# rsjahnige/CRYSTALS-Kyber

Hardware: AMD Instinct MI355X
Metric: ML-KEM-768 encaps+decaps/sec at batch 2^20; achieved HBM GB/s vs peak (higher is better)
Workload: dtype u32+f32 (64-bit Keccak lanes as 2 x u32; mod-3329 arithmetic exact on integers < 2^24 in the fp32 pipe; u8/u16 I/O)

## Files before the change

### crystals-kyber_amd/__init__.py

```python
import ctypes as C
import os

HERE = os.path.dirname(os.path.abspath(__file__))
LIB_PATH = os.environ.get("MLKEM_LIB_PATH") or os.path.join(HERE, "libmlkem_amd.so")
SHIM_PATH = os.path.join(HERE, "libml_kem.so")

SIZES = {512: (800, 1632, 768), 768: (1184, 2400, 1088), 1024: (1568, 3168, 1568)}
ERR_RNG = -2
ERR_MODULUS = -4
ERR_HASH = -5
ERR_KEY = -6
ERR_ARG = -101
KEYCHECK_EK_MODULUS = 1
KEYCHECK_DK_MODULUS = 2
KEYCHECK_DK_HASH = 4
KEYCHECK_EK_MISMATCH = 8
KEYCHECK_SEED = 16
KEYCHECK_PCT = 32

ABI_SYMBOLS = (
    "mlkem_sizes", "mlkem_params", "mlkem_device_count", "mlkem_strerror", "mlkem_last_hip_error",
    "mlkem_ctx_create", "mlkem_ctx_destroy", "mlkem_ctx_scratch_bytes", "mlkem_timing_begin", "mlkem_timing_end",
    "mlkem_keygen_dev", "mlkem_encaps_dev", "mlkem_decaps_dev", "mlkem_encaps_status_dev", "mlkem_ctx_set_conformance", "mlkem_ctx_debug_stages",
    "mlkem_encaps_shared_dev", "mlkem_decaps_shared_dev",
    "mlkem_pke_keygen_dev", "mlkem_pke_encrypt_dev", "mlkem_pke_decrypt_dev",
    "mlkem_ntt_dev", "mlkem_intt_dev", "mlkem_multiply_ntts_dev", "mlkem_sample_ntt_dev", "mlkem_sample_cbd_dev",
    "mlkem_compress_encode_dev", "mlkem_decode_decompress_dev",
    "mlkem_prf_dev", "mlkem_hash_dev", "mlkem_keccak_sponge_dev", "mlkem_sha3_pad_bits",
    "mlkem_keygen", "mlkem_encaps", "mlkem_decaps", "mlkem_ntt", "mlkem_intt", "mlkem_keccak_sponge",
    "mlkem_sample_ntt", "mlkem_sample_ntt_retries", "mlkem_sample_ntt_retries_dev", "mlkem_sample_cbd",
    "mlkem_keygen_random", "mlkem_encaps_random",
    "mlkem_cells_to_bytes_dev", "mlkem_bytes_to_cells_dev", "mlkem_keygen_stream", "mlkem_encaps_stream", "mlkem_decaps_stream", "mlkem_stream_release",
    "mlkem_compress_dev", "mlkem_decompress_dev", "mlkem_compress", "mlkem_decompress", "mlkem_sha3_pad_suffix",
    "mlkem_selftest_count", "mlkem_selftest", "mlkem_host_release", "mlkem_host_register", "mlkem_host_unregister",
    "mlkem_multi_create", "mlkem_multi_destroy", "mlkem_multi_members", "mlkem_multi_device", "mlkem_shard_range",
    "mlkem_keygen_multi", "mlkem_encaps_multi", "mlkem_decaps_multi",
    "mlkem_keygen_multi_dev", "mlkem_encaps_multi_dev", "mlkem_decaps_multi_dev", "mlkem_multi_sync", "mlkem_multi_stream", "mlkem_stream_last_staged",
    "mlkem_vector_multiply_dev", "mlkem_poly_add_dev", "mlkem_poly_sub_dev",
# ... 41 lines not shown
    L.mlkem_check_keys_dev.argtypes = [vp, i32, sz, vp, vp, vp, vp, vp, vp]
    L.mlkem_check_keys.argtypes = [i32, sz, vp, vp, vp, vp, vp]
    L.mlkem_keyset_create.argtypes = [vp, i32, sz, vp, vp, vp, vp, C.POINTER(vp), vp]
    L.mlkem_keyset_destroy.argtypes = [vp]
    L.mlkem_keyset_destroy.restype = None
    L.mlkem_keyset_info.argtypes = [vp, C.POINTER(i32), C.POINTER(sz), C.POINTER(i32), C.POINTER(sz)]
    L.mlkem_encaps_keyset_dev.argtypes = [vp, vp, sz, vp, vp, vp, vp, vp, vp]
    L.mlkem_decaps_keyset_dev.argtypes = [vp, vp, sz, vp, vp, vp, vp, vp]
    L.mlkem_ctx_rng_seed.argtypes = [vp, vp]
    L.mlkem_keygen_random_dev.argtypes = [vp, i32, sz, vp, vp, vp, vp]
    L.mlkem_encaps_random_dev.argtypes = [vp, i32, sz, vp, vp, vp, vp, vp]
    L.mlkem_encaps_keyset_random_dev.argtypes = [vp, vp, sz, vp, vp, vp, vp, vp]
    L.mlkem_encaps_status_dev.argtypes = [vp, i32, sz, vp, vp, vp, vp, vp, vp]
    L.mlkem_ctx_set_conformance.argtypes = [vp, i32]
    L.mlkem_ctx_debug_stages.argtypes = [vp, C.c_uint]
    L.mlkem_encaps_shared_dev.argtypes = [vp, i32, sz, vp, vp, vp, vp, vp]
    L.mlkem_decaps_shared_dev.argtypes = [vp, i32, sz, vp, vp, vp, vp, vp]
    L.mlkem_pke_keygen_dev.argtypes = [vp, i32, sz, vp, vp, vp, vp]
    L.mlkem_pke_encrypt_dev.argtypes = [vp, i32, sz, vp, vp, vp, vp, vp]
    L.mlkem_pke_decrypt_dev.argtypes = [vp, i32, sz, vp, vp, vp, vp]
    L.mlkem_ntt_dev.argtypes = [vp, sz, vp, vp, vp]
    L.mlkem_intt_dev.argtypes = [vp, sz, vp, vp, vp]
    L.mlkem_multiply_ntts_dev.argtypes = [vp, sz, vp, vp, vp, vp]
    L.mlkem_sample_ntt_dev.argtypes = [vp, sz, vp, vp, vp]
    L.mlkem_sample_cbd_dev.argtypes = [vp, i32, sz, vp, vp, vp]
    L.mlkem_prf_dev.argtypes = [vp, i32, sz, vp, vp, vp]
    L.mlkem_compress_encode_dev.argtypes = [vp, i32, sz, vp, vp, vp]
    L.mlkem_decode_decompress_dev.argtypes = [vp, i32, sz, vp, vp, vp]
    L.mlkem_hash_dev.argtypes = [vp, i32, sz, vp, C.c_uint, sz, vp, vp]
    L.mlkem_keygen.argtypes = [i32, sz, vp, vp, vp, vp]
# ... 125 lines not shown
        shape = (n,) if last is None else (n, last)
        if given is None:
            return torch.empty(shape, dtype=dtype, device=self.device)
        if not isinstance(given, torch.Tensor):
            raise MLKEMError(-101, "output must be a torch tensor")
        if given.device != self.device or given.dtype != dtype or tuple(given.shape) != shape or not given.is_contiguous():
            raise MLKEMError(-101, f"output tensor must be contiguous {dtype} {shape} on {self.device}, got "
                                   f"{given.dtype} {tuple(given.shape)} on {given.device}"
                                   f"{'' if given.is_contiguous() else ' (non-contiguous)'}")
        return given

    @property
    def scratch_bytes(self):
        return self.lib.mlkem_ctx_scratch_bytes(self._ctx)

    def keygen(self, d, z, ek=None, dk=None):
        u8 = self.torch.uint8
        d, z = self._dev(d, u8, 32), self._dev(z, u8, 32)
        n = d.shape[0]
        if z.shape[0] != n:
            raise MLKEMError(-101, "d and z batch sizes differ")
        ek = self._out(n, self.ek_len, given=ek)
        dk = self._out(n, self.dk_len, given=dk)
        self._check(self.lib.mlkem_keygen_dev(self._ctx, self.param_set, n, d.data_ptr(), z.data_ptr(), ek.data_ptr(),
                                              dk.data_ptr(), self._stream()))
        return ek, dk

    def encaps(self, ek, m, c=None, K=None, return_status=False):
        u8 = self.torch.uint8
        ek, m = self._dev(ek, u8, self.ek_len), self._dev(m, u8, 32)
# ... 577 lines not shown
```

### crystals-kyber_amd/csrc/mlkem_capi.hip

```cpp
#include "mlkem_pipeline.hpp"
#include "mlkem_keyset.hpp"
#include "mlkem_rng.hpp"
#include "mlkem_selftest.hpp"

#include "../../include/mlkem_batch.h"

#include <sys/random.h>

#include <cstdio>
#include <cstdlib>
#include <cstring>
#include <string.h>
#include <algorithm>
#include <condition_variable>
#include <functional>
#include <map>
#include <memory>
#include <mutex>
#include <new>
#include <string>
#include <thread>
#include <vector>

using namespace mlkem;
// ... 348 lines not shown
    return MLKEM_OK;
}
int mlkem_encaps_dev(mlkem_ctx* ctx, int set, size_t n, const uint8_t* ek, const uint8_t* m, uint8_t* c, uint8_t* K, void* stream) {
    return mlkem_encaps_status_dev(ctx, set, n, ek, m, c, K, nullptr, stream);
}

int mlkem_ctx_set_conformance(mlkem_ctx* ctx, int mode) {
    if (!ctx_ok(ctx) || (mode != MLKEM_CONFORMANCE_REFERENCE && mode != MLKEM_CONFORMANCE_FIPS203)) return MLKEM_ERR_ARG;
    ctx->ws.fips = mode == MLKEM_CONFORMANCE_FIPS203;
    return MLKEM_OK;
}

int mlkem_ctx_debug_stages(mlkem_ctx* ctx, unsigned mask) {
    if (!ctx_ok(ctx) || mask > 15u) return MLKEM_ERR_ARG;
    ctx->ws.stages = mask;
    return MLKEM_OK;
}

int mlkem_decaps_dev(mlkem_ctx* ctx, int set, size_t n, const uint8_t* dk, const uint8_t* c, uint8_t* K, int32_t* status, void* stream) {
    ParamSet p;
    if (!param_set(set, p)) return MLKEM_ERR_PARAM_SET;
    if (!ctx_ok(ctx) || (n && (!dk || !c || !K))) return MLKEM_ERR_ARG;
    if (!aligned16(dk) || !aligned16(c) || !aligned16(K) || (reinterpret_cast<uintptr_t>(status) & 3u)) return MLKEM_ERR_ARG;
    hipStream_t st = static_cast<hipStream_t>(stream);
    ctx_arm_side(ctx, n);
    decaps_dispatch(st, set, n, dk, c, K, status, status != nullptr, ctx->ws);
    HIP_TRY(hipGetLastError());
    return MLKEM_OK;
}

// ... 1421 lines not shown
```

### crystals-kyber_amd/csrc/mlkem_device.hpp

```cpp
#pragma once
#ifndef MLKEM_EMU
#include <hip/hip_runtime.h>
#endif
#include <stdint.h>

namespace mlkem {

constexpr int KQ = 3329;
constexpr int INV128 = 3303;

constexpr int cx_bitrev7(int r) {
    int o = 0;
    for (int i = 0; i < 7; i++) o |= ((r >> i) & 1) << (6 - i);
    return o;
}
constexpr int cx_pow17(int e) {
    int r = 1;
    for (int i = 0; i < e; i++) r = (r * 17) % KQ;
    return r;
}
constexpr int cx_centered(int x) { return x > KQ / 2 ? x - KQ : x; }
__device__ __forceinline__ unsigned div_q(unsigned num) {
    return (unsigned)(((uint64_t)num * 10321340ull) >> 35);
}
// ... 26 lines not shown
template <int N>
__device__ __forceinline__ void rotl64(uint32_t lo, uint32_t hi, uint32_t& olo, uint32_t& ohi) {
    if constexpr (N == 0) {
        olo = lo; ohi = hi;
    } else if constexpr (N < 32) {
        olo = __builtin_amdgcn_alignbit(lo, hi, 32 - N);
        ohi = __builtin_amdgcn_alignbit(hi, lo, 32 - N);
    } else if constexpr (N == 32) {
        olo = hi; ohi = lo;
    } else {
        olo = __builtin_amdgcn_alignbit(hi, lo, 64 - N);
        ohi = __builtin_amdgcn_alignbit(lo, hi, 64 - N);
    }
}

#define MLKEM_RHOPI(dst, src, rot, dx)                                                       \
    {                                                                                        \
        uint32_t tl = MLKEM_XOR3(s.lo[src], cl[(dx + 4) % 5], rl[(dx + 1) % 5]);             \
        uint32_t th = MLKEM_XOR3(s.hi[src], ch[(dx + 4) % 5], rh[(dx + 1) % 5]);             \
        rotl64<rot>(tl, th, bl[dst], bh[dst]);                                               \
    }

__device__ __forceinline__ void keccak_f1600(KeccakState& s) {
#pragma unroll 1
    for (int round = 0; round < 24; round++) {
        uint32_t cl[5], ch[5], rl[5], rh[5], bl[25], bh[25];
#pragma unroll
        for (int x = 0; x < 5; x++) {
            cl[x] = MLKEM_XOR3(MLKEM_XOR3(s.lo[x], s.lo[x + 5], s.lo[x + 10]), s.lo[x + 15], s.lo[x + 20]);
            ch[x] = MLKEM_XOR3(MLKEM_XOR3(s.hi[x], s.hi[x + 5], s.hi[x + 10]), s.hi[x + 15], s.hi[x + 20]);
        }
#pragma unroll
        for (int x = 0; x < 5; x++) rotl64<1>(cl[x], ch[x], rl[x], rh[x]);
        MLKEM_RHOPI(0, 0, 0, 0)   MLKEM_RHOPI(10, 1, 1, 1)  MLKEM_RHOPI(20, 2, 62, 2) MLKEM_RHOPI(5, 3, 28, 3)  MLKEM_RHOPI(15, 4, 27, 4)
        MLKEM_RHOPI(16, 5, 36, 0) MLKEM_RHOPI(1, 6, 44, 1)  MLKEM_RHOPI(11, 7, 6, 2)  MLKEM_RHOPI(21, 8, 55, 3) MLKEM_RHOPI(6, 9, 20, 4)
        MLKEM_RHOPI(7, 10, 3, 0)  MLKEM_RHOPI(17, 11, 10, 1) MLKEM_RHOPI(2, 12, 43, 2) MLKEM_RHOPI(12, 13, 25, 3) MLKEM_RHOPI(22, 14, 39, 4)
        MLKEM_RHOPI(23, 15, 41, 0) MLKEM_RHOPI(8, 16, 45, 1) MLKEM_RHOPI(18, 17, 15, 2) MLKEM_RHOPI(3, 18, 21, 3) MLKEM_RHOPI(13, 19, 8, 4)
        MLKEM_RHOPI(14, 20, 18, 0) MLKEM_RHOPI(24, 21, 2, 1) MLKEM_RHOPI(9, 22, 61, 2) MLKEM_RHOPI(19, 23, 56, 3) MLKEM_RHOPI(4, 24, 14, 4)
#pragma unroll
        for (int y = 0; y < 25; y += 5) {
#pragma unroll
            for (int x = 0; x < 5; x++) {
                s.lo[y + x] = MLKEM_CHI(bl[y + x], bl[y + (x + 1) % 5], bl[y + (x + 2) % 5]);
                s.hi[y + x] = MLKEM_CHI(bh[y + x], bh[y + (x + 1) % 5], bh[y + (x + 2) % 5]);
            }
        }
        s.lo[0] ^= KECCAK_RC[2 * round];
        s.hi[0] ^= KECCAK_RC[2 * round + 1];
    }
}

__device__ __forceinline__ void keccak_zero(KeccakState& s) {
#pragma unroll
    for (int i = 0; i < 25; i++) { s.lo[i] = 0; s.hi[i] = 0; }
}

template <int POS>
__device__ __forceinline__ void keccak_xor_byte(KeccakState& s, uint32_t byte) {
    constexpr int w = POS / 4, sh = 8 * (POS % 4);
    if constexpr (w % 2 == 0) s.lo[w / 2] ^= byte << sh;
    else s.hi[w / 2] ^= byte << sh;
}
template <int W>
// ... 178 lines not shown
```

### crystals-kyber_amd/csrc/mlkem_kernels.hpp

```cpp
#pragma once
#include "mlkem_device.hpp"

namespace mlkem {

constexpr int WAVE = 64;

#ifndef MLKEM_KECCAK_MINWAVES
#define MLKEM_KECCAK_MINWAVES 6
#endif

struct MsgView {
    const uint8_t* p0; size_t stride0; unsigned len0;
    const uint8_t* p1; size_t stride1; unsigned len1;
};

__device__ __forceinline__ uint2 load_qword_tail(const uint8_t* p, unsigned avail) {
    if (avail >= 8) return *reinterpret_cast<const uint2*>(p);
    uint2 v;
    v.x = 0; v.y = 0;
    for (unsigned i = 0; i < avail; i++) {
        const uint32_t b = p[i];
        if (i < 4) v.x |= b << (8 * i);
        else v.y |= b << (8 * (i - 4));
    }
// ... 143 lines not shown
}

__device__ __forceinline__ void keccak_xor_byte_rt(KeccakState& s, unsigned pos, uint32_t byte) {
    const unsigned w = pos >> 2;
    const uint32_t v = byte << (8 * (pos & 3));
#define MLKEM_XB(W) keccak_word<W>(s) ^= (w == W) ? v : 0u;
    MLKEM_XB(0) MLKEM_XB(1) MLKEM_XB(2) MLKEM_XB(3) MLKEM_XB(4) MLKEM_XB(5) MLKEM_XB(6) MLKEM_XB(7)
    MLKEM_XB(8) MLKEM_XB(9) MLKEM_XB(10) MLKEM_XB(11) MLKEM_XB(12) MLKEM_XB(13) MLKEM_XB(14) MLKEM_XB(15)
    MLKEM_XB(16) MLKEM_XB(17) MLKEM_XB(18) MLKEM_XB(19) MLKEM_XB(20) MLKEM_XB(21) MLKEM_XB(22) MLKEM_XB(23)
    MLKEM_XB(24) MLKEM_XB(25) MLKEM_XB(26) MLKEM_XB(27) MLKEM_XB(28) MLKEM_XB(29) MLKEM_XB(30) MLKEM_XB(31)
    MLKEM_XB(32) MLKEM_XB(33) MLKEM_XB(34) MLKEM_XB(35) MLKEM_XB(36) MLKEM_XB(37) MLKEM_XB(38) MLKEM_XB(39)
    MLKEM_XB(40) MLKEM_XB(41)
#undef MLKEM_XB
}

template <int RATE, int SUFFIX>
__device__ __forceinline__ void wave_sponge_absorb(KeccakState& s, uint2* stage, const MsgView& mv, size_t item0,
                                                   size_t n_items) {
    const unsigned total = mv.len0 + mv.len1;
    keccak_zero(s);
#if MLKEM_STAGE_DMA
    if (item0 + WAVE <= n_items && total != 0 && total % 4 == 0 && (mv.len1 == 0 || mv.len0 % 16 == 0) &&
        mv.stride0 < (1u << 27) && mv.stride1 < (1u << 27)) {
        uint32_t* st32 = reinterpret_cast<uint32_t*>(stage);
        const unsigned nfull = total / (unsigned)RATE, rem = total - nfull * (unsigned)RATE;
        wave_dma_half<RATE>(st32, mv, item0, 0, nfull ? (unsigned)RATE : rem, 0);
#pragma unroll 1
        for (unsigned b = 0; b < nfull; b++) {
            wave_absorb_dma<RATE, true>(s, st32, mv, item0, b * RATE, RATE);
            if (b + 1 < nfull) wave_dma_half<RATE>(st32, mv, item0, (b + 1) * RATE, RATE, 0);
            else if (rem) wave_dma_half<RATE>(st32, mv, item0, nfull * RATE, rem, 0);
            keccak_f1600(s);
        }
        if (rem) wave_absorb_dma<RATE, false>(s, st32, mv, item0, nfull * RATE, rem);
        keccak_xor_byte_rt(s, rem, SUFFIX);
        keccak_xor_byte<RATE - 1>(s, 0x80);
        keccak_f1600(s);
        return;
    }
#endif
    unsigned voff = 0;
    while (total - voff >= (unsigned)RATE) {
        wave_absorb_block<RATE>(s, stage, mv, item0, n_items, voff);
        keccak_f1600(s);
        voff += RATE;
    }
    const unsigned rem = total - voff;
    if (rem) wave_absorb_block<RATE>(s, stage, mv, item0, n_items, voff);
    keccak_xor_byte_rt(s, rem, SUFFIX);
    keccak_xor_byte<RATE - 1>(s, 0x80);
    keccak_f1600(s);
}

constexpr int stage_qwords(int max_rate) {
    const int sync_q = STAGE_ROWS * (max_rate / 8);
    const int dma_q = MLKEM_STAGE_DMA ? 2 * ((max_rate / 4 + 3) / 4) * WAVE / 2 : 0;
    return sync_q > dma_q ? sync_q : dma_q;
}
constexpr int STAGE_QWORDS = stage_qwords(168);

__device__ __forceinline__ void store32(uint8_t* base, size_t stride, size_t item, const uint32_t (&w)[8]) {
    uint32_t* p = reinterpret_cast<uint32_t*>(base + item * stride);
#pragma unroll
    for (int i = 0; i < 8; i++) p[i] = w[i];
}
__device__ __forceinline__ void load32(const uint8_t* base, size_t stride, size_t item, uint32_t (&w)[8]) {
// ... 2 lines not shown
    for (int i = 0; i < 8; i++) w[i] = p[i];
}
#define MLKEM_STATE_WORDS8(s, FIRST, w)                                                             \
    {                                                                                               \
        w[0] = keccak_word<FIRST + 0>(s); w[1] = keccak_word<FIRST + 1>(s); w[2] = keccak_word<FIRST + 2>(s); \
        w[3] = keccak_word<FIRST + 3>(s); w[4] = keccak_word<FIRST + 4>(s); w[5] = keccak_word<FIRST + 5>(s); \
        w[6] = keccak_word<FIRST + 6>(s); w[7] = keccak_word<FIRST + 7>(s);                         \
    }
#define MLKEM_SET_WORDS8(s, FIRST, w)                                                               \
    {                                                                                               \
        keccak_word<FIRST + 0>(s) = w[0]; keccak_word<FIRST + 1>(s) = w[1]; keccak_word<FIRST + 2>(s) = w[2]; \
        keccak_word<FIRST + 3>(s) = w[3]; keccak_word<FIRST + 4>(s) = w[4]; keccak_word<FIRST + 5>(s) = w[5]; \
        keccak_word<FIRST + 6>(s) = w[6]; keccak_word<FIRST + 7>(s) = w[7];                         \
    }

__device__ __forceinline__ void lane_G64(KeccakState& s, const uint32_t (&x)[8], const uint32_t (&y)[8]) {
    keccak_zero(s);
    MLKEM_SET_WORDS8(s, 0, x)
    MLKEM_SET_WORDS8(s, 8, y)
    keccak_xor_byte<64>(s, 0x06);
    keccak_xor_byte<71>(s, 0x80);
    keccak_f1600(s);
}

template <int K>
__global__ void __launch_bounds__(WAVE, MLKEM_KECCAK_MINWAVES) k_hash_encaps(size_t n, const uint8_t* __restrict__ ek, const uint8_t* __restrict__ m,
                                                      uint8_t* __restrict__ Kout, uint8_t* __restrict__ r_ws) {
    __shared__ __attribute__((aligned(16))) uint2 stage[stage_qwords(136)];
    constexpr unsigned EK = 384 * K + 32;
    const size_t item0 = (size_t)blockIdx.x * WAVE, item = item0 + lane_id();
    KeccakState s;
    MsgView mv{ek, EK, EK, ek, EK, 0};
    wave_sponge_absorb<136, 0x06>(s, stage, mv, item0, n);
    uint32_t h[8], mm[8], w[8];
    MLKEM_STATE_WORDS8(s, 0, h)
    const size_t it = item < n ? item : n - 1;
    load32(m, 32, it, mm);
    lane_G64(s, mm, h);
    if (item < n) {
        MLKEM_STATE_WORDS8(s, 0, w)
        store32(Kout, 32, item, w);
        MLKEM_STATE_WORDS8(s, 8, w)
        store32(r_ws, 32, item, w);
    }
}

__global__ void __launch_bounds__(WAVE, MLKEM_KECCAK_MINWAVES) k_hash_g_shared(size_t n, const uint8_t* __restrict__ m, const uint8_t* __restrict__ h,
                                                                               uint8_t* __restrict__ Kout, uint8_t* __restrict__ r_ws) {
    const size_t item = (size_t)blockIdx.x * WAVE + lane_id();
    const size_t it = item < n ? item : n - 1;
    uint32_t mm[8], hh[8], w[8];
    load32(m, 32, it, mm);
    load32(h, 0, 0, hh);
// ... 31 lines not shown
                                                      int32_t* __restrict__ status, size_t dk_stride) {
    __shared__ __attribute__((aligned(16))) uint2 stage[STAGE_QWORDS];
    constexpr unsigned EK = 384 * K + 32;
    const size_t DK = dk_stride;
    const size_t nb = (n + WAVE - 1) / WAVE;
    const bool check_role = HASH_CHECK && blockIdx.x < nb;
    const size_t item0 = (size_t)(HASH_CHECK && !check_role ? blockIdx.x - nb : blockIdx.x) * WAVE;
    KeccakState s;
    uint32_t h[8], w[8];
    auto my_item = [&]() {
        const size_t i2 = item0 + (size_t)lane_id_fresh();
        return i2 < n ? i2 : n - 1;
    };
    if (check_role) {
        MsgView mv{dk + 384 * K, DK, EK, dk, DK, 0};
        wave_sponge_absorb<136, 0x06>(s, stage, mv, item0, n);
        MLKEM_STATE_WORDS8(s, 0, w)
        load32(dk + 768 * K + 32, DK, my_item(), h);
        uint32_t diff = 0;
#pragma unroll
        for (int i = 0; i < 8; i++) diff |= w[i] ^ h[i];
        const size_t i2 = item0 + (size_t)lane_id_fresh();
        if (i2 < n && status) status[i2] = diff ? -5 : 0;
        return;
    }
    {
        MsgView mv{dk + 768 * K + 64, DK, 32, c, CLEN, CLEN};
        wave_sponge_absorb<JRATE, 0x1F>(s, stage, mv, item0, n);
        const size_t i2 = item0 + (size_t)lane_id_fresh();
        if (i2 < n) {
            MLKEM_STATE_WORDS8(s, 0, w)
            store32(Kbar_ws, 32, i2, w);
        }
    }
    uint32_t mm[8];
    const size_t it = my_item();
    load32(m_ws, 32, it, mm);
    load32(dk + 768 * K + 32, DK, it, h);
    lane_G64(s, mm, h);
    const size_t item = item0 + (size_t)lane_id_fresh();
    if (item < n) {
        MLKEM_STATE_WORDS8(s, 0, w)
        store32(Kp_ws, 32, item, w);
        MLKEM_STATE_WORDS8(s, 8, w)
        store32(r_ws, 32, item, w);
        if (!HASH_CHECK && status) status[item] = 0;
    }
}

template <int K>
__global__ void __launch_bounds__(WAVE, MLKEM_KECCAK_MINWAVES) k_hash_keygen_seed(size_t n, const uint8_t* __restrict__ d, uint8_t* __restrict__ rho_ws,
                                                           uint8_t* __restrict__ sigma_ws) {
    const size_t item = (size_t)blockIdx.x * WAVE + lane_id();
    const size_t it = item < n ? item : n - 1;
// ... 296 lines not shown
```

### crystals-kyber_amd/csrc/mlkem_sampler.hpp

```cpp
#pragma once
#include "mlkem_kernels.hpp"

namespace mlkem {

constexpr int LIN_STRIDE = 144;
#ifdef MLKEM_EMU
#define MLKEM_LIN_ACCEPT(lds0, pos, d) { if ((d) < (uint32_t)QB) { *reinterpret_cast<int16_t*>((lds0) + (pos)) = (int16_t)(d); (pos) += 2u; } }
#define MLKEM_LIN_ACCEPT_LIM(lds0, pos, d, lim) { if ((d) < (uint32_t)QB && (pos) < (lim)) { *reinterpret_cast<int16_t*>((lds0) + (pos)) = (int16_t)(d); (pos) += 2u; } }
#else
#define MLKEM_LIN_ACCEPT(lds0, pos, d)                                              \
    asm volatile("v_cmpx_gt_u32 vcc, 0xd01, %1\n\t"                                 \
                 "ds_write_b16 %0, %1\n\t"                                          \
                 "v_add_u32 %0, 2, %0\n\t"                                          \
                 "s_mov_b64 exec, -1"                                               \
                 : "+v"(pos) : "v"(d) : "vcc", "memory")
#define MLKEM_LIN_ACCEPT_LIM(lds0, pos, d, lim)                                     \
    asm volatile("v_cmpx_gt_u32 vcc, 0xd01, %1\n\t"                                 \
                 "v_cmpx_gt_u32 vcc, %2, %0\n\t"                                    \
                 "ds_write_b16 %0, %1\n\t"                                          \
                 "v_add_u32 %0, 2, %0\n\t"                                          \
                 "s_mov_b64 exec, -1"                                               \
                 : "+v"(pos) : "v"(d), "v"(lim) : "vcc", "memory")
#endif
#define MLKEM_LG(ACC, W0, FIRST, LAST)                                                                         \
    {                                                                                                           \
        const uint32_t w0 = keccak_word<W0>(s), w1 = keccak_word<W0 + 1>(s), w2 = keccak_word<W0 + 2>(s);       \
        if (FIRST <= 0 && LAST > 0) { ACC(w0 & 0xFFFu) ACC((w0 >> 12) & 0xFFFu) }                               \
        if (FIRST <= 1 && LAST > 1) { ACC(__builtin_amdgcn_alignbit(w1, w0, 24) & 0xFFFu) ACC((w1 >> 4) & 0xFFFu) } \
        if (FIRST <= 2 && LAST > 2) { ACC((w1 >> 16) & 0xFFFu) ACC(__builtin_amdgcn_alignbit(w2, w1, 28) & 0xFFFu) } \
        if (FIRST <= 3 && LAST > 3) { ACC((w2 >> 8) & 0xFFFu) ACC(w2 >> 20) }                                   \
    }
#define MLKEM_LBLOCK(ACC, FLUSH)                                                                               \
    MLKEM_LG(ACC, 0, 0, 4) MLKEM_LG(ACC, 3, 0, 4) MLKEM_LG(ACC, 6, 0, 4) MLKEM_LG(ACC, 9, 0, 4)                 \
    MLKEM_LG(ACC, 12, 0, 4) MLKEM_LG(ACC, 15, 0, 4) MLKEM_LG(ACC, 18, 0, 4)                                     \
    FLUSH                                                                                                       \
    MLKEM_LG(ACC, 21, 0, 4) MLKEM_LG(ACC, 24, 0, 4) MLKEM_LG(ACC, 27, 0, 4) MLKEM_LG(ACC, 30, 0, 4)             \
    MLKEM_LG(ACC, 33, 0, 4) MLKEM_LG(ACC, 36, 0, 4) MLKEM_LG(ACC, 39, 0, 4)                                     \
    FLUSH

__device__ __forceinline__ void lin_flush(char* buf, uint32_t pos0, uint32_t& pos, uint32_t& lim, uint32_t& flushed, char* dst_poly, bool valid) {
    const uint32_t n32 = (pos - pos0) >> 5;
#pragma unroll
    for (uint32_t i = 0; i < 4; i++)
        if (i < n32 && valid) {
            const uint4 a = *reinterpret_cast<const uint4*>(buf + 32u * i), b = *reinterpret_cast<const uint4*>(buf + 32u * i + 16u);
            stream_store16(dst_poly + flushed + 32u * i, a);
            stream_store16(dst_poly + flushed + 32u * i + 16u, b);
        }
    if (n32) {
        const uint4 a = *reinterpret_cast<const uint4*>(buf + 32u * n32);
        *reinterpret_cast<uint4*>(buf) = a;
        if (n32 < 4) {
            const uint4 b = *reinterpret_cast<const uint4*>(buf + 32u * n32 + 16u);
            *reinterpret_cast<uint4*>(buf + 16u) = b;
        }
    }
    pos -= 32u * n32;
    lim -= 32u * n32;
    flushed += 32u * n32;
}

template <int QB = KQ>
__global__ void __launch_bounds__(WAVE, 4) k_sample_main(SampleArgs a) {
#ifndef MLKEM_EMU
// ... 21 lines not shown
        uint32_t resume_cnt = 0;
        {
            char* lbuf = stage + l * LIN_STRIDE;
#ifdef MLKEM_EMU
            char* const lds0 = lbuf;
            const uint32_t pos0 = 0;
#else
            const uint32_t pos0 = (uint32_t)reinterpret_cast<uintptr_t>(lbuf);
#endif
            uint32_t pos = pos0, lim = pos0 + 512u, flushed = 0;
            char* dst_poly = reinterpret_cast<char*>(a.A + gc * 256);
            const bool valid = g < a.n_xof;
#define MLKEM_ACC_FAST(d) { const uint32_t dd = (d); MLKEM_LIN_ACCEPT(lds0, pos, dd); }
#define MLKEM_ACC_LIM(d) { const uint32_t dd = (d); MLKEM_LIN_ACCEPT_LIM(lds0, pos, dd, lim); }
#define MLKEM_LFLUSH { wave_lds_fence(); lin_flush(lbuf, pos0, pos, lim, flushed, dst_poly, valid); wave_lds_fence(); }
            keccak_f1600(s);
            MLKEM_LBLOCK(MLKEM_ACC_FAST, MLKEM_LFLUSH)
            keccak_f1600(s);
            MLKEM_LBLOCK(MLKEM_ACC_FAST, MLKEM_LFLUSH)
            keccak_f1600(s);
            MLKEM_LBLOCK(MLKEM_ACC_LIM, MLKEM_LFLUSH)
#undef MLKEM_ACC_FAST
#undef MLKEM_ACC_LIM
#undef MLKEM_LFLUSH
            unfinished = flushed < 512u;
            if (unfinished && valid) {
                *reinterpret_cast<uint4*>(dst_poly + flushed) = *reinterpret_cast<const uint4*>(lbuf);
                *reinterpret_cast<uint4*>(dst_poly + flushed + 16u) = *reinterpret_cast<const uint4*>(lbuf + 16);
            }
            resume_cnt = (flushed + (pos - pos0)) >> 1;
        }
        if (unfinished && g < a.n_xof) {
            const uint32_t idx = atomicAdd(&a.leftover[1], 1u);
            if (idx < a.resume_cap) {
                uint32_t* e = a.resume + (size_t)idx * RESUME_WORDS;
                e[0] = (uint32_t)g;
                e[1] = resume_cnt;
#define MLKEM_SV(W) e[2 + W] = keccak_word<W>(s);
                MLKEM_SV(0) MLKEM_SV(1) MLKEM_SV(2) MLKEM_SV(3) MLKEM_SV(4) MLKEM_SV(5) MLKEM_SV(6) MLKEM_SV(7) MLKEM_SV(8) MLKEM_SV(9)
// ... 9 lines not shown
        }
    } else {
        const size_t g = (size_t)(blockIdx.x - a.xof_blocks) * WAVE + l;
        const size_t gc = g < a.n_prf ? g : a.n_prf - 1;
        uint32_t seed[8];
        const size_t item = gc / (size_t)a.per_item;
        const unsigned ctr = (unsigned)(gc - item * (size_t)a.per_item);
        load32(a.r, 32, item, seed);
        const unsigned eta = (int)ctr < a.n_eta1 ? (unsigned)a.eta1 : 2u;
        keccak_zero(s);
        MLKEM_SET_WORDS8(s, 0, seed)
        keccak_xor_byte<32>(s, ctr);
        keccak_xor_byte<33>(s, 0x1F);
        if (a.prf_rate == 136) keccak_xor_byte<135>(s, 0x80);
        else keccak_xor_byte<167>(s, 0x80);
        keccak_f1600(s);
        uint32_t* st32 = reinterpret_cast<uint32_t*>(stage);
        const size_t g0 = g - (size_t)l;
#pragma unroll 1
        for (int half = 0; half < 2; half++) {
            if ((l >> 5) == half) {
                uint32_t* mine = st32 + (l & 31) * 33;
#define MLKEM_SW(W) mine[W] = keccak_word<W>(s);
                MLKEM_SW(0) MLKEM_SW(1) MLKEM_SW(2) MLKEM_SW(3) MLKEM_SW(4) MLKEM_SW(5) MLKEM_SW(6) MLKEM_SW(7)
                MLKEM_SW(8) MLKEM_SW(9) MLKEM_SW(10) MLKEM_SW(11) MLKEM_SW(12) MLKEM_SW(13) MLKEM_SW(14) MLKEM_SW(15)
                MLKEM_SW(16) MLKEM_SW(17) MLKEM_SW(18) MLKEM_SW(19) MLKEM_SW(20) MLKEM_SW(21) MLKEM_SW(22) MLKEM_SW(23)
                MLKEM_SW(24) MLKEM_SW(25) MLKEM_SW(26) MLKEM_SW(27) MLKEM_SW(28) MLKEM_SW(29) MLKEM_SW(30) MLKEM_SW(31)
#undef MLKEM_SW
            }
            wave_lds_fence();
#pragma unroll
// ... 64 lines not shown
```

### include/mlkem_batch.h

```cpp
#ifndef MLKEM_BATCH_H
#define MLKEM_BATCH_H

#include <stddef.h>
#include <stdint.h>

#ifndef MLKEM_API
#define MLKEM_API __attribute__((visibility("default")))
#endif

#ifdef __cplusplus
extern "C" {
#endif

#define MLKEM_OK 0
#define MLKEM_ERR_PARAM_SET (-1)
#define MLKEM_ERR_RNG (-2)
#define MLKEM_ERR_LENGTH (-3)
#define MLKEM_ERR_MODULUS (-4)
#define MLKEM_ERR_HASH (-5)
#define MLKEM_ERR_KEY (-6)
#define MLKEM_ERR_NO_DEVICE (-100)
#define MLKEM_ERR_ARG (-101)
#define MLKEM_ERR_ALLOC (-102)

// ... 1 lines not shown
MLKEM_API int mlkem_params(int param_set, int out_k_eta1_eta2_du_dv[5]);
MLKEM_API int mlkem_device_count(void);
MLKEM_API const char* mlkem_strerror(int code);
MLKEM_API const char* mlkem_last_hip_error(void);

typedef struct mlkem_ctx mlkem_ctx;
MLKEM_API int mlkem_ctx_create(mlkem_ctx** out, int device, size_t chunk_items);
MLKEM_API void mlkem_ctx_destroy(mlkem_ctx* ctx);
MLKEM_API size_t mlkem_ctx_scratch_bytes(const mlkem_ctx* ctx);

#define MLKEM_CONFORMANCE_REFERENCE 0
#define MLKEM_CONFORMANCE_FIPS203 1
MLKEM_API int mlkem_ctx_set_conformance(mlkem_ctx* ctx, int mode);

MLKEM_API int mlkem_ctx_debug_stages(mlkem_ctx* ctx, unsigned mask);
MLKEM_API int mlkem_timing_begin(void);
MLKEM_API int mlkem_timing_end(char* labels, double* total_ms, int* counts, int max);

MLKEM_API int mlkem_keygen_dev(mlkem_ctx* ctx, int param_set, size_t n, const uint8_t* d, const uint8_t* z, uint8_t* ek, uint8_t* dk,
                     void* stream);
MLKEM_API int mlkem_encaps_dev(mlkem_ctx* ctx, int param_set, size_t n, const uint8_t* ek, const uint8_t* m, uint8_t* c, uint8_t* K,
                     void* stream);
MLKEM_API int mlkem_encaps_status_dev(mlkem_ctx* ctx, int param_set, size_t n, const uint8_t* ek, const uint8_t* m, uint8_t* c, uint8_t* K,
                            int32_t* status, void* stream);
MLKEM_API int mlkem_decaps_dev(mlkem_ctx* ctx, int param_set, size_t n, const uint8_t* dk, const uint8_t* c, uint8_t* K, int32_t* status,
                     void* stream);
MLKEM_API int mlkem_decaps_seed_dev(mlkem_ctx* ctx, int param_set, size_t n, const uint8_t* seed, const uint8_t* c, uint8_t* K, void* stream);

#define MLKEM_KEYCHECK_EK_MODULUS 1
#define MLKEM_KEYCHECK_DK_MODULUS 2
// ... 115 lines not shown
```

Baseline: 62.21 million.

## Specialize Keccak first/last rounds for known-zero input and partial-output lanes

Adds Keccak-f1600 variants that skip theta/chi work for lanes that are known zero in the first round and for output lanes that are never read in the last round. These are applied to the G/H hashes, the PRF and the SampleNTT first squeeze. The final SampleNTT block drops the per-accept limit check in favour of a clamped flush. A debug leftover-count API is also added. The goal is fewer ALU ops in the Keccak-bound stages, at the cost of more template code paths and correctness risk if the zero or needed-lane masks are wrong.

```diff
diff --git a/crystals-kyber_amd/__init__.py b/crystals-kyber_amd/__init__.py
--- a/crystals-kyber_amd/__init__.py
+++ b/crystals-kyber_amd/__init__.py
@@ -22,6 +22,7 @@
     "mlkem_sizes", "mlkem_params", "mlkem_device_count", "mlkem_strerror", "mlkem_last_hip_error",
     "mlkem_ctx_create", "mlkem_ctx_destroy", "mlkem_ctx_scratch_bytes", "mlkem_timing_begin", "mlkem_timing_end",
     "mlkem_keygen_dev", "mlkem_encaps_dev", "mlkem_decaps_dev", "mlkem_encaps_status_dev", "mlkem_ctx_set_conformance", "mlkem_ctx_debug_stages",
+    "mlkem_ctx_debug_leftover",
     "mlkem_encaps_shared_dev", "mlkem_decaps_shared_dev",
     "mlkem_pke_keygen_dev", "mlkem_pke_encrypt_dev", "mlkem_pke_decrypt_dev",
     "mlkem_ntt_dev", "mlkem_intt_dev", "mlkem_multiply_ntts_dev", "mlkem_sample_ntt_dev", "mlkem_sample_cbd_dev",
@@ -93,6 +94,7 @@
     L.mlkem_encaps_status_dev.argtypes = [vp, i32, sz, vp, vp, vp, vp, vp, vp]
     L.mlkem_ctx_set_conformance.argtypes = [vp, i32]
     L.mlkem_ctx_debug_stages.argtypes = [vp, C.c_uint]
+    L.mlkem_ctx_debug_leftover.argtypes = [vp, C.POINTER(C.c_uint32), vp]
     L.mlkem_encaps_shared_dev.argtypes = [vp, i32, sz, vp, vp, vp, vp, vp]
     L.mlkem_decaps_shared_dev.argtypes = [vp, i32, sz, vp, vp, vp, vp, vp]
     L.mlkem_pke_keygen_dev.argtypes = [vp, i32, sz, vp, vp, vp, vp]
@@ -248,6 +250,11 @@
     def scratch_bytes(self):
         return self.lib.mlkem_ctx_scratch_bytes(self._ctx)
 
+    def debug_leftover(self):
+        v = (C.c_uint32 * 2)()
+        self._check(self.lib.mlkem_ctx_debug_leftover(self._ctx, v, self._stream()))
+        return int(v[0]), int(v[1])
+
     def keygen(self, d, z, ek=None, dk=None):
         u8 = self.torch.uint8
         d, z = self._dev(d, u8, 32), self._dev(z, u8, 32)
diff --git a/crystals-kyber_amd/csrc/mlkem_capi.hip b/crystals-kyber_amd/csrc/mlkem_capi.hip
--- a/crystals-kyber_amd/csrc/mlkem_capi.hip
+++ b/crystals-kyber_amd/csrc/mlkem_capi.hip
@@ -386,6 +386,17 @@
 int mlkem_ctx_debug_stages(mlkem_ctx* ctx, unsigned mask) {
     if (!ctx_ok(ctx) || mask > 15u) return MLKEM_ERR_ARG;
     ctx->ws.stages = mask;
+    return MLKEM_OK;
+}
+
+int mlkem_ctx_debug_leftover(mlkem_ctx* ctx, uint32_t counts[2], void* stream) {
+    if (!ctx_ok(ctx) || !counts) return MLKEM_ERR_ARG;
+    hipStream_t st = static_cast<hipStream_t>(stream);
+    uint32_t v[2] = {0, 0};
+    HIP_TRY(hipMemcpyAsync(v, ctx->ws.leftover, sizeof(v), hipMemcpyDeviceToHost, st));
+    HIP_TRY(hipStreamSynchronize(st));
+    counts[0] = v[1];
+    counts[1] = v[0];
     return MLKEM_OK;
 }
 
diff --git a/crystals-kyber_amd/csrc/mlkem_device.hpp b/crystals-kyber_amd/csrc/mlkem_device.hpp
--- a/crystals-kyber_amd/csrc/mlkem_device.hpp
+++ b/crystals-kyber_amd/csrc/mlkem_device.hpp
@@ -64,39 +64,155 @@
     }
 }
 
-#define MLKEM_RHOPI(dst, src, rot, dx)                                                       \
-    {                                                                                        \
+#ifndef MLKEM_TRIM
+#define MLKEM_TRIM 7
+#endif
+
+#define MLKEM_RHOPI(NEED, dst, src, rot, dx)                                                 \
+    if constexpr (keccak_need_b(NEED, dst)) {                                                \
         uint32_t tl = MLKEM_XOR3(s.lo[src], cl[(dx + 4) % 5], rl[(dx + 1) % 5]);             \
         uint32_t th = MLKEM_XOR3(s.hi[src], ch[(dx + 4) % 5], rh[(dx + 1) % 5]);             \
         rotl64<rot>(tl, th, bl[dst], bh[dst]);                                               \
     }
+constexpr bool keccak_need_b(int need, int b) {
+    const int y = b / 5 * 5, x = b % 5;
+    return y + x < need || y + (x + 4) % 5 < need || y + (x + 3) % 5 < need;
+}
+
+#define MLKEM_KECCAK_ROUND(NEED)                                                                                             \
+    {                                                                                                                        \
+        uint32_t cl[5], ch[5], rl[5], rh[5], bl[25], bh[25];                                                                 \
+                      \
+        _Pragma("unroll")                                                                                                    \
+        for (int x = 0; x < 5; x++) {                                                                                        \
+            cl[x] = MLKEM_XOR3(MLKEM_XOR3(s.lo[x], s.lo[x + 5], s.lo[x + 10]), s.lo[x + 15], s.lo[x + 20]);                  \
+            ch[x] = MLKEM_XOR3(MLKEM_XOR3(s.hi[x], s.hi[x + 5], s.hi[x + 10]), s.hi[x + 15], s.hi[x + 20]);                  \
+        }                                                                                                                    \
+        _Pragma("unroll")                                                                                                    \
+        for (int x = 0; x < 5; x++) rotl64<1>(cl[x], ch[x], rl[x], rh[x]);                                                   \
+                     \
+        MLKEM_RHOPI(NEED, 0, 0, 0, 0)   MLKEM_RHOPI(NEED, 10, 1, 1, 1)  MLKEM_RHOPI(NEED, 20, 2, 62, 2)                      \
+        MLKEM_RHOPI(NEED, 5, 3, 28, 3)  MLKEM_RHOPI(NEED, 15, 4, 27, 4)                                                      \
+        MLKEM_RHOPI(NEED, 16, 5, 36, 0) MLKEM_RHOPI(NEED, 1, 6, 44, 1)  MLKEM_RHOPI(NEED, 11, 7, 6, 2)                       \
+        MLKEM_RHOPI(NEED, 21, 8, 55, 3) MLKEM_RHOPI(NEED, 6, 9, 20, 4)                                                       \
+        MLKEM_RHOPI(NEED, 7, 10, 3, 0)  MLKEM_RHOPI(NEED, 17, 11, 10, 1) MLKEM_RHOPI(NEED, 2, 12, 43, 2)                     \
+        MLKEM_RHOPI(NEED, 12, 13, 25, 3) MLKEM_RHOPI(NEED, 22, 14, 39, 4)                                                    \
+        MLKEM_RHOPI(NEED, 23, 15, 41, 0) MLKEM_RHOPI(NEED, 8, 16, 45, 1) MLKEM_RHOPI(NEED, 18, 17, 15, 2)                    \
+        MLKEM_RHOPI(NEED, 3, 18, 21, 3) MLKEM_RHOPI(NEED, 13, 19, 8, 4)                                                      \
+        MLKEM_RHOPI(NEED, 14, 20, 18, 0) MLKEM_RHOPI(NEED, 24, 21, 2, 1) MLKEM_RHOPI(NEED, 9, 22, 61, 2)                     \
+        MLKEM_RHOPI(NEED, 19, 23, 56, 3) MLKEM_RHOPI(NEED, 4, 24, 14, 4)                                                     \
+                                                                                                   \
+        _Pragma("unroll")                                                                                                    \
+        for (int y = 0; y < 25; y += 5) {                                                                                    \
+            _Pragma("unroll")                                                                                                \
+            for (int x = 0; x < 5; x++) {                                                                                    \
+                if (NEED >= 25 || y + x < NEED) {               \
+                    s.lo[y + x] = MLKEM_CHI(bl[y + x], bl[y + (x + 1) % 5], bl[y + (x + 2) % 5]);                            \
+                    s.hi[y + x] = MLKEM_CHI(bh[y + x], bh[y + (x + 1) % 5], bh[y + (x + 2) % 5]);                            \
+                }                                                                                                            \
+            }                                                                                                                \
+        }                                                                                                                    \
+                                                                                                  \
+        s.lo[0] ^= KECCAK_RC[2 * round];                                                                                     \
+        s.hi[0] ^= KECCAK_RC[2 * round + 1];                                                                                 \
+    }
 
 __device__ __forceinline__ void keccak_f1600(KeccakState& s) {
 #pragma unroll 1
-    for (int round = 0; round < 24; round++) {
-        uint32_t cl[5], ch[5], rl[5], rh[5], bl[25], bh[25];
+    for (int round = 0; round < 24; round++) MLKEM_KECCAK_ROUND(25)
+}
+__device__ __forceinline__ void keccak_rounds(KeccakState& s, int first, int last) {
+#pragma unroll 1
+    for (int round = first; round < last; round++) MLKEM_KECCAK_ROUND(25)
+}
+template <int NEED>
+__device__ __forceinline__ void keccak_round_last(KeccakState& s) {
+    static_assert(NEED >= 1 && NEED <= 25, "lanes");
+    constexpr int round = 23;
+    MLKEM_KECCAK_ROUND(NEED)
+}
+
+template <int NEED>
+__device__ __forceinline__ void keccak_f1600(KeccakState& s) {
+    if constexpr (NEED >= 25 || !(MLKEM_TRIM & 2)) {
+        keccak_rounds(s, 0, 24);
+    } else {
+        keccak_rounds(s, 0, 23);
+        keccak_round_last<NEED>(s);
+    }
+}
+
+constexpr uint32_t keccak_zero_except(uint32_t nonzero) { return ~nonzero & 0x1FFFFFFu; }
+constexpr int keccak_col_count(uint32_t zero, int x) {
+    int n = 0;
+    for (int y = 0; y < 5; y++) n += !((zero >> (x + 5 * y)) & 1u);
+    return n;
+}
+constexpr int keccak_col_lane(uint32_t zero, int x, int j) {
+    for (int y = 0; y < 5; y++)
+        if (!((zero >> (x + 5 * y)) & 1u) && j-- == 0) return x + 5 * y;
+    return 0;
+}
+template <uint32_t ZERO, int X>
+__device__ __forceinline__ uint32_t keccak_col_parity(const uint32_t (&a)[25]) {
+    constexpr int n = keccak_col_count(ZERO, X);
+    constexpr int i0 = keccak_col_lane(ZERO, X, 0), i1 = keccak_col_lane(ZERO, X, 1), i2 = keccak_col_lane(ZERO, X, 2),
+                  i3 = keccak_col_lane(ZERO, X, 3), i4 = keccak_col_lane(ZERO, X, 4);
+    if constexpr (n == 0) return 0u;
+    else if constexpr (n == 1) return a[i0];
+    else if constexpr (n == 2) return a[i0] ^ a[i1];
+    else if constexpr (n == 3) return MLKEM_XOR3(a[i0], a[i1], a[i2]);
+    else if constexpr (n == 4) return MLKEM_XOR3(a[i0], a[i1], a[i2]) ^ a[i3];
+    else return MLKEM_XOR3(MLKEM_XOR3(a[i0], a[i1], a[i2]), a[i3], a[i4]);
+}
+#define MLKEM_RHOPI0(dst, src, rot, dx)                                                      \
+    {                                                                                        \
+        if constexpr ((ZERO >> src) & 1u) rotl64<rot>(dl[dx], dh[dx], bl[dst], bh[dst]);     \
+        else rotl64<rot>(s.lo[src] ^ dl[dx], s.hi[src] ^ dh[dx], bl[dst], bh[dst]);          \
+    }
+template <uint32_t ZERO>
+__device__ __forceinline__ void keccak_round_first(KeccakState& s) {
+    uint32_t cl[5], ch[5], dl[5], dh[5], bl[25], bh[25];
+    cl[0] = keccak_col_parity<ZERO, 0>(s.lo); ch[0] = keccak_col_parity<ZERO, 0>(s.hi);
+    cl[1] = keccak_col_parity<ZERO, 1>(s.lo); ch[1] = keccak_col_parity<ZERO, 1>(s.hi);
+    cl[2] = keccak_col_parity<ZERO, 2>(s.lo); ch[2] = keccak_col_parity<ZERO, 2>(s.hi);
+    cl[3] = keccak_col_parity<ZERO, 3>(s.lo); ch[3] = keccak_col_parity<ZERO, 3>(s.hi);
+    cl[4] = keccak_col_parity<ZERO, 4>(s.lo); ch[4] = keccak_col_parity<ZERO, 4>(s.hi);
+#pragma unroll
+    for (int x = 0; x < 5; x++) {
+        uint32_t rl, rh;
+        rotl64<1>(cl[(x + 1) % 5], ch[(x + 1) % 5], rl, rh);
+        dl[x] = cl[(x + 4) % 5] ^ rl;
+        dh[x] = ch[(x + 4) % 5] ^ rh;
+    }
+    MLKEM_RHOPI0(0, 0, 0, 0)   MLKEM_RHOPI0(10, 1, 1, 1)  MLKEM_RHOPI0(20, 2, 62, 2) MLKEM_RHOPI0(5, 3, 28, 3)  MLKEM_RHOPI0(15, 4, 27, 4)
+    MLKEM_RHOPI0(16, 5, 36, 0) MLKEM_RHOPI0(1, 6, 44, 1)  MLKEM_RHOPI0(11, 7, 6, 2)  MLKEM_RHOPI0(21, 8, 55, 3) MLKEM_RHOPI0(6, 9, 20, 4)
+    MLKEM_RHOPI0(7, 10, 3, 0)  MLKEM_RHOPI0(17, 11, 10, 1) MLKEM_RHOPI0(2, 12, 43, 2) MLKEM_RHOPI0(12, 13, 25, 3) MLKEM_RHOPI0(22, 14, 39, 4)
+    MLKEM_RHOPI0(23, 15, 41, 0) MLKEM_RHOPI0(8, 16, 45, 1) MLKEM_RHOPI0(18, 17, 15, 2) MLKEM_RHOPI0(3, 18, 21, 3) MLKEM_RHOPI0(13, 19, 8, 4)
+    MLKEM_RHOPI0(14, 20, 18, 0) MLKEM_RHOPI0(24, 21, 2, 1) MLKEM_RHOPI0(9, 22, 61, 2) MLKEM_RHOPI0(19, 23, 56, 3) MLKEM_RHOPI0(4, 24, 14, 4)
+#pragma unroll
+    for (int y = 0; y < 25; y += 5) {
 #pragma unroll
         for (int x = 0; x < 5; x++) {
-            cl[x] = MLKEM_XOR3(MLKEM_XOR3(s.lo[x], s.lo[x + 5], s.lo[x + 10]), s.lo[x + 15], s.lo[x + 20]);
-            ch[x] = MLKEM_XOR3(MLKEM_XOR3(s.hi[x], s.hi[x + 5], s.hi[x + 10]), s.hi[x + 15], s.hi[x + 20]);
+            s.lo[y + x] = MLKEM_CHI(bl[y + x], bl[y + (x + 1) % 5], bl[y + (x + 2) % 5]);
+            s.hi[y + x] = MLKEM_CHI(bh[y + x], bh[y + (x + 1) % 5], bh[y + (x + 2) % 5]);
         }
-#pragma unroll
-        for (int x = 0; x < 5; x++) rotl64<1>(cl[x], ch[x], rl[x], rh[x]);
-        MLKEM_RHOPI(0, 0, 0, 0)   MLKEM_RHOPI(10, 1, 1, 1)  MLKEM_RHOPI(20, 2, 62, 2) MLKEM_RHOPI(5, 3, 28, 3)  MLKEM_RHOPI(15, 4, 27, 4)
-        MLKEM_RHOPI(16, 5, 36, 0) MLKEM_RHOPI(1, 6, 44, 1)  MLKEM_RHOPI(11, 7, 6, 2)  MLKEM_RHOPI(21, 8, 55, 3) MLKEM_RHOPI(6, 9, 20, 4)
-        MLKEM_RHOPI(7, 10, 3, 0)  MLKEM_RHOPI(17, 11, 10, 1) MLKEM_RHOPI(2, 12, 43, 2) MLKEM_RHOPI(12, 13, 25, 3) MLKEM_RHOPI(22, 14, 39, 4)
-        MLKEM_RHOPI(23, 15, 41, 0) MLKEM_RHOPI(8, 16, 45, 1) MLKEM_RHOPI(18, 17, 15, 2) MLKEM_RHOPI(3, 18, 21, 3) MLKEM_RHOPI(13, 19, 8, 4)
-        MLKEM_RHOPI(14, 20, 18, 0) MLKEM_RHOPI(24, 21, 2, 1) MLKEM_RHOPI(9, 22, 61, 2) MLKEM_RHOPI(19, 23, 56, 3) MLKEM_RHOPI(4, 24, 14, 4)
-#pragma unroll
-        for (int y = 0; y < 25; y += 5) {
-#pragma unroll
-            for (int x = 0; x < 5; x++) {
-                s.lo[y + x] = MLKEM_CHI(bl[y + x], bl[y + (x + 1) % 5], bl[y + (x + 2) % 5]);
-                s.hi[y + x] = MLKEM_CHI(bh[y + x], bh[y + (x + 1) % 5], bh[y + (x + 2) % 5]);
-            }
-        }
-        s.lo[0] ^= KECCAK_RC[2 * round];
-        s.hi[0] ^= KECCAK_RC[2 * round + 1];
+    }
+    s.lo[0] ^= 0x00000001u;
+}
+template <uint32_t ZERO, int NEED = 25>
+__device__ __forceinline__ void keccak_f1600_first(KeccakState& s, bool all_lanes = false) {
+    int from = 0;
+    if constexpr ((MLKEM_TRIM & 1) != 0) {
+        keccak_round_first<ZERO>(s);
+        from = 1;
+    }
+    if constexpr (NEED >= 25 || !(MLKEM_TRIM & 2)) {
+        keccak_rounds(s, from, 24);
+    } else {
+        keccak_rounds(s, from, 23);
+        if (all_lanes) keccak_round_last<25>(s);
+        else keccak_round_last<NEED>(s);
     }
 }
 
diff --git a/crystals-kyber_amd/csrc/mlkem_kernels.hpp b/crystals-kyber_amd/csrc/mlkem_kernels.hpp
--- a/crystals-kyber_amd/csrc/mlkem_kernels.hpp
+++ b/crystals-kyber_amd/csrc/mlkem_kernels.hpp
@@ -181,7 +181,7 @@
 #undef MLKEM_XB
 }
 
-template <int RATE, int SUFFIX>
+template <int RATE, int SUFFIX, int NEED = 25>
 __device__ __forceinline__ void wave_sponge_absorb(KeccakState& s, uint2* stage, const MsgView& mv, size_t item0,
                                                    size_t n_items) {
     const unsigned total = mv.len0 + mv.len1;
@@ -202,7 +202,7 @@
         if (rem) wave_absorb_dma<RATE, false>(s, st32, mv, item0, nfull * RATE, rem);
         keccak_xor_byte_rt(s, rem, SUFFIX);
         keccak_xor_byte<RATE - 1>(s, 0x80);
-        keccak_f1600(s);
+        keccak_f1600<NEED>(s);
         return;
     }
 #endif
@@ -216,7 +216,7 @@
     if (rem) wave_absorb_block<RATE>(s, stage, mv, item0, n_items, voff);
     keccak_xor_byte_rt(s, rem, SUFFIX);
     keccak_xor_byte<RATE - 1>(s, 0x80);
-    keccak_f1600(s);
+    keccak_f1600<NEED>(s);
 }
 
 constexpr int stage_qwords(int max_rate) {
@@ -249,13 +249,15 @@
         keccak_word<FIRST + 6>(s) = w[6]; keccak_word<FIRST + 7>(s) = w[7];                         \
     }
 
+template <bool TRIM = false>
 __device__ __forceinline__ void lane_G64(KeccakState& s, const uint32_t (&x)[8], const uint32_t (&y)[8]) {
     keccak_zero(s);
     MLKEM_SET_WORDS8(s, 0, x)
     MLKEM_SET_WORDS8(s, 8, y)
     keccak_xor_byte<64>(s, 0x06);
     keccak_xor_byte<71>(s, 0x80);
-    keccak_f1600(s);
+    if constexpr (TRIM) keccak_f1600_first<keccak_zero_except(0x1FFu), 8>(s);
+    else keccak_f1600(s);
 }
 
 template <int K>
@@ -266,12 +268,12 @@
     const size_t item0 = (size_t)blockIdx.x * WAVE, item = item0 + lane_id();
     KeccakState s;
     MsgView mv{ek, EK, EK, ek, EK, 0};
-    wave_sponge_absorb<136, 0x06>(s, stage, mv, item0, n);
+    wave_sponge_absorb<136, 0x06, 4>(s, stage, mv, item0, n);
     uint32_t h[8], mm[8], w[8];
     MLKEM_STATE_WORDS8(s, 0, h)
     const size_t it = item < n ? item : n - 1;
     load32(m, 32, it, mm);
-    lane_G64(s, mm, h);
+    lane_G64<true>(s, mm, h);
     if (item < n) {
         MLKEM_STATE_WORDS8(s, 0, w)
         store32(Kout, 32, item, w);
@@ -333,7 +335,7 @@
     };
     if (check_role) {
         MsgView mv{dk + 384 * K, DK, EK, dk, DK, 0};
-        wave_sponge_absorb<136, 0x06>(s, stage, mv, item0, n);
+        wave_sponge_absorb<136, 0x06, 4>(s, stage, mv, item0, n);
         MLKEM_STATE_WORDS8(s, 0, w)
         load32(dk + 768 * K + 32, DK, my_item(), h);
         uint32_t diff = 0;
@@ -345,7 +347,7 @@
     }
     {
         MsgView mv{dk + 768 * K + 64, DK, 32, c, CLEN, CLEN};
-        wave_sponge_absorb<JRATE, 0x1F>(s, stage, mv, item0, n);
+        wave_sponge_absorb<JRATE, 0x1F, 4>(s, stage, mv, item0, n);
         const size_t i2 = item0 + (size_t)lane_id_fresh();
         if (i2 < n) {
             MLKEM_STATE_WORDS8(s, 0, w)
@@ -356,7 +358,7 @@
     const size_t it = my_item();
     load32(m_ws, 32, it, mm);
     load32(dk + 768 * K + 32, DK, it, h);
-    lane_G64(s, mm, h);
+    lane_G64<true>(s, mm, h);
     const size_t item = item0 + (size_t)lane_id_fresh();
     if (item < n) {
         MLKEM_STATE_WORDS8(s, 0, w)
diff --git a/crystals-kyber_amd/csrc/mlkem_sampler.hpp b/crystals-kyber_amd/csrc/mlkem_sampler.hpp
--- a/crystals-kyber_amd/csrc/mlkem_sampler.hpp
+++ b/crystals-kyber_amd/csrc/mlkem_sampler.hpp
@@ -6,7 +6,9 @@
 constexpr int LIN_STRIDE = 144;
 #ifdef MLKEM_EMU
 #define MLKEM_LIN_ACCEPT(lds0, pos, d) { if ((d) < (uint32_t)QB) { *reinterpret_cast<int16_t*>((lds0) + (pos)) = (int16_t)(d); (pos) += 2u; } }
+#if !(MLKEM_TRIM & 4)
 #define MLKEM_LIN_ACCEPT_LIM(lds0, pos, d, lim) { if ((d) < (uint32_t)QB && (pos) < (lim)) { *reinterpret_cast<int16_t*>((lds0) + (pos)) = (int16_t)(d); (pos) += 2u; } }
+#endif
 #else
 #define MLKEM_LIN_ACCEPT(lds0, pos, d)                                              \
     asm volatile("v_cmpx_gt_u32 vcc, 0xd01, %1\n\t"                                 \
@@ -14,6 +16,7 @@
                  "v_add_u32 %0, 2, %0\n\t"                                          \
                  "s_mov_b64 exec, -1"                                               \
                  : "+v"(pos) : "v"(d) : "vcc", "memory")
+#if !(MLKEM_TRIM & 4)
 #define MLKEM_LIN_ACCEPT_LIM(lds0, pos, d, lim)                                     \
     asm volatile("v_cmpx_gt_u32 vcc, 0xd01, %1\n\t"                                 \
                  "v_cmpx_gt_u32 vcc, %2, %0\n\t"                                    \
@@ -22,6 +25,7 @@
                  "s_mov_b64 exec, -1"                                               \
                  : "+v"(pos) : "v"(d), "v"(lim) : "vcc", "memory")
 #endif
+#endif
 #define MLKEM_LG(ACC, W0, FIRST, LAST)                                                                         \
     {                                                                                                           \
         const uint32_t w0 = keccak_word<W0>(s), w1 = keccak_word<W0 + 1>(s), w2 = keccak_word<W0 + 2>(s);       \
@@ -38,8 +42,18 @@
     MLKEM_LG(ACC, 33, 0, 4) MLKEM_LG(ACC, 36, 0, 4) MLKEM_LG(ACC, 39, 0, 4)                                     \
     FLUSH
 
+template <bool CLAMP = false>
 __device__ __forceinline__ void lin_flush(char* buf, uint32_t pos0, uint32_t& pos, uint32_t& lim, uint32_t& flushed, char* dst_poly, bool valid) {
-    const uint32_t n32 = (pos - pos0) >> 5;
+    uint32_t n32 = (pos - pos0) >> 5;
+    bool keep = true;
+    if constexpr (CLAMP) {
+        const uint32_t room = (512u - flushed) >> 5;
+        if (n32 >= room) {
+            n32 = room;
+            pos = pos0 + 32u * n32;
+            keep = false;
+        }
+    }
 #pragma unroll
     for (uint32_t i = 0; i < 4; i++)
         if (i < n32 && valid) {
@@ -47,7 +61,7 @@
             stream_store16(dst_poly + flushed + 32u * i, a);
             stream_store16(dst_poly + flushed + 32u * i + 16u, b);
         }
-    if (n32) {
+    if (n32 && keep) {
         const uint4 a = *reinterpret_cast<const uint4*>(buf + 32u * n32);
         *reinterpret_cast<uint4*>(buf) = a;
         if (n32 < 4) {
@@ -99,15 +113,21 @@
 #define MLKEM_ACC_FAST(d) { const uint32_t dd = (d); MLKEM_LIN_ACCEPT(lds0, pos, dd); }
 #define MLKEM_ACC_LIM(d) { const uint32_t dd = (d); MLKEM_LIN_ACCEPT_LIM(lds0, pos, dd, lim); }
 #define MLKEM_LFLUSH { wave_lds_fence(); lin_flush(lbuf, pos0, pos, lim, flushed, dst_poly, valid); wave_lds_fence(); }
-            keccak_f1600(s);
+#define MLKEM_LFLUSH_CLAMP { wave_lds_fence(); lin_flush<true>(lbuf, pos0, pos, lim, flushed, dst_poly, valid); wave_lds_fence(); }
+            keccak_f1600_first<keccak_zero_except(0x10001Fu)>(s);
             MLKEM_LBLOCK(MLKEM_ACC_FAST, MLKEM_LFLUSH)
             keccak_f1600(s);
             MLKEM_LBLOCK(MLKEM_ACC_FAST, MLKEM_LFLUSH)
             keccak_f1600(s);
+#if MLKEM_TRIM & 4
+            MLKEM_LBLOCK(MLKEM_ACC_FAST, MLKEM_LFLUSH_CLAMP)
+#else
             MLKEM_LBLOCK(MLKEM_ACC_LIM, MLKEM_LFLUSH)
+#endif
 #undef MLKEM_ACC_FAST
 #undef MLKEM_ACC_LIM
 #undef MLKEM_LFLUSH
+#undef MLKEM_LFLUSH_CLAMP
             unfinished = flushed < 512u;
             if (unfinished && valid) {
                 *reinterpret_cast<uint4*>(dst_poly + flushed) = *reinterpret_cast<const uint4*>(lbuf);
@@ -147,7 +167,7 @@
         keccak_xor_byte<33>(s, 0x1F);
         if (a.prf_rate == 136) keccak_xor_byte<135>(s, 0x80);
         else keccak_xor_byte<167>(s, 0x80);
-        keccak_f1600(s);
+        keccak_f1600_first<keccak_zero_except(0x11001Fu), 16>(s, a.eta1 == 3);
         uint32_t* st32 = reinterpret_cast<uint32_t*>(stage);
         const size_t g0 = g - (size_t)l;
 #pragma unroll 1
diff --git a/include/mlkem_batch.h b/include/mlkem_batch.h
--- a/include/mlkem_batch.h
+++ b/include/mlkem_batch.h
@@ -39,6 +39,7 @@
 MLKEM_API int mlkem_ctx_set_conformance(mlkem_ctx* ctx, int mode);
 
 MLKEM_API int mlkem_ctx_debug_stages(mlkem_ctx* ctx, unsigned mask);
+MLKEM_API int mlkem_ctx_debug_leftover(mlkem_ctx* ctx, uint32_t counts[2], void* stream);
 MLKEM_API int mlkem_timing_begin(void);
 MLKEM_API int mlkem_timing_end(char* labels, double* total_ms, int* counts, int max);
 
```

Result: no change. 62.82 million, median of 6 (+1.0%).
